# golmschenk/sr-gan

Hardware: AMD Instinct MI355X
Metric: SRGAN train images/sec (G+D step) (higher is better)
Workload: dtype f32; 1 GPU; crowd SRGAN (KnnDenseNetCat D/DNN + DCGenerator) 512x512, batch 16/GPU, dnn_training_step + gan_training_step per step; global_batch=16, image_size=512, schedule=shared-forwards, parallelism=dp1, random_init_weights=True, gradient_penalty=active, launch=eager (Python tape enqueues every kernel), schedule_check=not run: the --full option runs it

## Files before the change

include/srgan_hip.h:

```cpp
#ifndef SRGAN_HIP_H
#define SRGAN_HIP_H

#include <stdint.h>

#ifdef __cplusplus
extern "C" {
#endif

int srgan_version(void);
const char* srgan_build_id(void);
const char* srgan_last_error(void);

#define SRGAN_DTYPE_F32 0x1u
#define SRGAN_DTYPE_BF16 0x2u
#define SRGAN_DTYPE_F16 0x4u
#define SRGAN_FEATURE_FUSED_BNRELU 0x1u
#define SRGAN_FEATURE_SPLITK_WORKSPACE 0x2u
#define SRGAN_FEATURE_LIVE_PROFILE 0x4u
#define SRGAN_FEATURE_BLOCKED16 0x8u
#define SRGAN_FEATURE_BATCHED_SHADOWS 0x10u
#define SRGAN_FEATURE_CROWD_FULL_IMAGE 0x20u
#define SRGAN_FEATURE_IMAGE_BATCHES 0x40u
#define SRGAN_FEATURE_BATCH_NORM_TRAIN 0x80u
#define SRGAN_FEATURE_BLOCKED_BATCH_NORM 0x100u
#define SRGAN_FEATURE_BLOCKED_FROZEN_NORM 0x200u
typedef struct srgan_capabilities_t {
  int32_t abi_version;
  int32_t struct_bytes;
  char arch[16];
  uint32_t dtypes;
  uint32_t features;
  int64_t workspace_bytes;
  int64_t max_tensor_elements;
} srgan_capabilities_t;
int srgan_capabilities(srgan_capabilities_t* out, int32_t out_bytes);
int64_t srgan_workspace_bytes(void);
int srgan_set_workspace(void* workspace, int64_t bytes, void* stream);
int srgan_split_is_ordered(void* stream);

typedef struct srgan_conv_desc {
  int32_t N, C, H, W;
  int32_t K, R, S;
  int32_t stride_h, stride_w, pad_h, pad_w;
  int32_t OH, OW;
  int64_t x_batch_stride, y_batch_stride;
  int32_t compute_dtype;
} srgan_conv_desc;

#define SRGAN_COMPUTE_F32 0
#define SRGAN_COMPUTE_BF16 1
#define SRGAN_COMPUTE_F16 2

int srgan_conv2d_fwd(const srgan_conv_desc* desc, const float* x, const float* w, const float* bias, float* y,
                     int force_kernel, void* stream);

int srgan_conv2d_bwd_data(const srgan_conv_desc* desc, const float* gy, const float* w, const float* bias, float* gx,
                          int accumulate, int force_kernel, void* stream);

// ... 184 lines not shown
int64_t srgan_h_k4s2_weight_slots(int32_t A, int32_t B, int direction, int dtype);
int srgan_h_pack_k4s2_weights(const float* w, void* packed, int32_t A, int32_t B, int direction, int dtype, void* stream);
int32_t srgan_h_pack_job_bytes(void);
int64_t srgan_h_pack_job_conv_weights(void* jobs, int64_t first_block, const float* w, void* packed, int32_t K, int32_t C, int32_t R,
                                      int32_t S, int transposed, int dtype);
int64_t srgan_h_pack_job_k4s2_weights(void* jobs, int64_t first_block, const float* w, void* packed, int32_t A, int32_t B,
                                      int direction, int dtype, int32_t* jobs_written);
int64_t srgan_h_pack_job_matrix(void* jobs, int64_t first_block, const float* src, void* out, int64_t rows, int64_t cols,
                                int64_t rows_real, int64_t cols_real, int64_t row_stride, int64_t col_stride, int32_t row_plane,
                                int32_t col_plane, int dtype);
int64_t srgan_h_pack_job_bias_rows(void* jobs, int64_t first_block, const float* bias, float* rows, int32_t channels, int32_t plane);
int srgan_h_pack_batched(const void* jobs_device, int32_t count, int64_t blocks, void* stream);
int srgan_h_conv4x4s2(const void* x, const void* packed, const float* bias, const void* ref, float slope, int epi, void* out,
                      int32_t N, int32_t C_in, int32_t rows, int32_t H, int32_t W, int dtype, void* stream);
int srgan_h_conv_transpose4x4s2(const void* x, const void* packed, const float* bias, const void* ref, float slope, int epi,
                                void* out, int32_t N, int32_t C_in, int32_t rows, int32_t h, int32_t w, int dtype, void* stream);
int srgan_h_k4s2_wgrad(const void* big, const void* small, float* gw, int32_t N, int32_t C_big, int32_t C_small, int32_t H, int32_t W,
                       int small_is_rows, int dtype, void* stream);

int srgan_h_batch_norm_stats(const void* x, float* mean, float* inv_std, float* running_mean, float* running_var,
                             int64_t* num_batches_tracked, float momentum, float eps, int32_t N, int32_t C, int64_t HW,
                             int32_t dtype, void* stream);
int srgan_h_batch_norm_fwd(const void* x, const float* mean, const float* inv_std, const float* gamma, const float* beta,
                           float slope, void* y, int32_t N, int32_t C, int64_t HW, int32_t dtype, void* stream);
int srgan_h_batch_norm_bwd_reduce(const void* s, const void* x, const float* mean, const float* inv_std, float* sums,
                                  float* g_gamma, float* g_beta, int32_t N, int32_t C, int64_t HW, int32_t dtype, void* stream);
int srgan_h_batch_norm_bwd_apply(const void* s, const void* x, const float* mean, const float* inv_std, const float* gamma,
                                 const float* sums, const void* ref, float slope, void* gx, int32_t N, int32_t C, int64_t HW,
                                 int32_t dtype, void* stream);
int srgan_h_frozen_norm_bwd(const void* s, const void* x, const float* mean, const float* inv_std, const float* gamma,
                            const void* ref, float slope, void* gx, float* g_gamma, float* g_beta, int32_t N, int32_t C, int64_t HW,
                            int32_t dtype, void* stream);

int srgan_profile_begin(void);
int srgan_profile_end(double* kernel_ms, double* flops, double* mfma_flops, int64_t* launches);
int srgan_profile_bytes(double* algorithmic_bytes_total);
int srgan_profile_mixed(double* flops, double* kernel_ms);
int64_t srgan_profile_report(char* buffer, int64_t capacity);

#ifdef __cplusplus
}
#endif
#endif
```

sr-gan_amd/_lib.py:

```python
import ctypes
import os

from ._build import LIBRARY, source_id

c_float_p = ctypes.c_void_p
i32, i64, f32, vp = ctypes.c_int32, ctypes.c_int64, ctypes.c_float, ctypes.c_void_p


class ConvDesc(ctypes.Structure):
    _fields_ = [(name, i32) for name in ('N', 'C', 'H', 'W', 'K', 'R', 'S', 'stride_h', 'stride_w', 'pad_h', 'pad_w',
                                         'OH', 'OW')] + [('x_batch_stride', i64), ('y_batch_stride', i64), ('compute_dtype', i32)]


class BnRelu(ctypes.Structure):
    _fields_ = [(name, vp) for name in ('mean', 'inv_std', 'gamma', 'beta')]


class BnReduceJob(ctypes.Structure):
    _fields_ = [('partial_offset', i64), ('tiles', i32), ('channels', i32), ('inv_std', vp), ('g_gamma', vp), ('g_beta', vp)]


class Capabilities(ctypes.Structure):
    _fields_ = [('abi_version', i32), ('struct_bytes', i32), ('arch', ctypes.c_char * 16), ('dtypes', ctypes.c_uint32),
                ('features', ctypes.c_uint32), ('workspace_bytes', i64), ('max_tensor_elements', i64)]
# ... 84 lines not shown
    'srgan_adam_step': ([vp, vp, vp, vp, i64, f32, f32, f32, f32, f32, i32, vp], ctypes.c_int),
    'srgan_adam_step_counted': ([vp, vp, vp, vp, i64, f32, f32, f32, f32, f32, vp, vp], ctypes.c_int),
    'srgan_pack_bf16': ([vp, vp, i64, vp], ctypes.c_int),
    'srgan_unpack_bf16': ([vp, vp, i64, vp], ctypes.c_int),
    'srgan_h_pack': ([vp, vp, vp, f32, i32, i32, i64, ctypes.c_int, vp], ctypes.c_int),
    'srgan_h_unpack': ([vp, vp, i32, i32, i64, ctypes.c_int, vp], ctypes.c_int),
    'srgan_h_add': ([vp, vp, vp, i64, ctypes.c_int, vp], ctypes.c_int),
    'srgan_h_channel_sums': ([vp, vp, i32, i32, i64, ctypes.c_int, vp], ctypes.c_int),
    'srgan_h_maxpool2': ([vp, vp, vp, i64, i32, i32, ctypes.c_int, ctypes.c_int, vp], ctypes.c_int),
    'srgan_h_maxpool2_bwd': ([vp, vp, vp, i64, i32, i32, ctypes.c_int, f32, ctypes.c_int, vp], ctypes.c_int),
    'srgan_h_conv_weight_slots': ([i32, i32, i32, i32], ctypes.c_int64),
    'srgan_h_pack_conv_weights': ([vp, vp, i32, i32, i32, i32, ctypes.c_int, ctypes.c_int, vp], ctypes.c_int),
    'srgan_h_conv3x3': ([vp, vp, vp, vp, f32, ctypes.c_int, vp, i32, i32, i32, i32, i32, i32, ctypes.c_int, vp], ctypes.c_int),
    'srgan_h_conv3x3_wgrad': ([vp, vp, vp, i32, i32, i32, i32, i32, ctypes.c_int, vp], ctypes.c_int),
    'srgan_h_pack_matrix': ([vp, vp, i64, i64, i64, i64, i64, i64, i32, i32, ctypes.c_int, vp], ctypes.c_int),
    'srgan_h_gemm': ([vp, vp, vp, vp, f32, ctypes.c_int, vp, i32, i32, i32, i32, i32, ctypes.c_int, vp], ctypes.c_int),
    'srgan_h_linear_wgrad': ([vp, vp, vp, i32, i32, i32, i64, i64, i64, i64, i32, i32, ctypes.c_int, vp], ctypes.c_int),
    'srgan_h_k4s2_weight_slots': ([i32, i32, ctypes.c_int, ctypes.c_int], ctypes.c_int64),
    'srgan_h_pack_k4s2_weights': ([vp, vp, i32, i32, ctypes.c_int, ctypes.c_int, vp], ctypes.c_int),
    'srgan_h_pack_job_bytes': ([], ctypes.c_int32),
    'srgan_h_pack_job_conv_weights': ([vp, i64, vp, vp, i32, i32, i32, i32, ctypes.c_int, ctypes.c_int], ctypes.c_int64),
    'srgan_h_pack_job_k4s2_weights': ([vp, i64, vp, vp, i32, i32, ctypes.c_int, ctypes.c_int, vp], ctypes.c_int64),
    'srgan_h_pack_job_matrix': ([vp, i64, vp, vp, i64, i64, i64, i64, i64, i64, i32, i32, ctypes.c_int], ctypes.c_int64),
    'srgan_h_pack_job_bias_rows': ([vp, i64, vp, vp, i32, i32], ctypes.c_int64),
    'srgan_h_pack_batched': ([vp, i32, i64, vp], ctypes.c_int),
    'srgan_h_conv4x4s2': ([vp, vp, vp, vp, f32, ctypes.c_int, vp, i32, i32, i32, i32, i32, ctypes.c_int, vp], ctypes.c_int),
    'srgan_h_conv_transpose4x4s2': ([vp, vp, vp, vp, f32, ctypes.c_int, vp, i32, i32, i32, i32, i32, ctypes.c_int, vp], ctypes.c_int),
    'srgan_h_k4s2_wgrad': ([vp, vp, vp, i32, i32, i32, i32, i32, ctypes.c_int, ctypes.c_int, vp], ctypes.c_int),
    'srgan_h_batch_norm_stats': ([vp, vp, vp, vp, vp, vp, f32, f32, i32, i32, i64, i32, vp], ctypes.c_int),
    'srgan_h_batch_norm_fwd': ([vp, vp, vp, vp, vp, f32, vp, i32, i32, i64, i32, vp], ctypes.c_int),
    'srgan_h_batch_norm_bwd_reduce': ([vp, vp, vp, vp, vp, vp, vp, i32, i32, i64, i32, vp], ctypes.c_int),
    'srgan_h_batch_norm_bwd_apply': ([vp, vp, vp, vp, vp, vp, vp, f32, vp, i32, i32, i64, i32, vp], ctypes.c_int),
    'srgan_h_frozen_norm_bwd': ([vp, vp, vp, vp, vp, vp, f32, vp, vp, vp, i32, i32, i64, i32, vp], ctypes.c_int),
    'srgan_comm_available': ([], ctypes.c_int),
    'srgan_comm_unique_id': ([vp], ctypes.c_int),
    'srgan_comm_init': ([ctypes.POINTER(vp), i32, i32, vp], ctypes.c_int),
    'srgan_comm_world_size': ([vp, ctypes.POINTER(i32)], ctypes.c_int),
    'srgan_comm_destroy': ([vp], ctypes.c_int),
    'srgan_all_reduce_sum': ([vp, vp, vp, i64, i32, vp], ctypes.c_int),
    'srgan_reduce_scatter_sum': ([vp, vp, vp, i64, i32, vp], ctypes.c_int),
    'srgan_all_gather': ([vp, vp, vp, i64, i32, vp], ctypes.c_int),
    'srgan_broadcast': ([vp, vp, i64, i32, i32, vp], ctypes.c_int),
}


EINVAL, EUNSUPPORTED, ERANGE = -1, -2, -3


class HipLibraryError(RuntimeError):

    def __init__(self, message, status=None):
        super().__init__(message)
        self.status = status


_library = None


def library():
    global _library
    if _library is None:
        if not os.path.exists(LIBRARY):
            raise HipLibraryError(f'{LIBRARY} is missing: run `python -c "import __graft_entry__ as g; g.build()"` '
                                  '(there is no CPU fallback)')
        import torch
        lib = ctypes.CDLL(LIBRARY)
# ... 42 lines not shown
```

sr-gan_amd/crowd/models.py:

```python
from collections import OrderedDict

from torch import nn as torch_nn

from .. import functional as F
from .. import nn
from .. import fused
from ..age.models import Generator as _DCGANGenerator, convolution, LEAK
from ..utility import seed_all


FUSED_STEM_POOL = True


class DCGenerator(_DCGANGenerator):

    def __init__(self, z_dim=256, image_size=224, conv_dim=64, batch_norm=None, blocked_batch_norm=False):
        super().__init__(z_dim=z_dim, image_size=image_size, conv_dim=conv_dim, batch_norm=batch_norm,
                         blocked_batch_norm=blocked_batch_norm)


class JointDCDiscriminator(nn.Module):

    def __init__(self, image_size=128, conv_dim=64, number_of_outputs=1):
        seed_all(0)
        super().__init__()
        self.number_of_outputs = number_of_outputs
        self.layer1 = convolution(3, conv_dim, 4, bn=False)
        self.layer2 = convolution(conv_dim, conv_dim * 2, 4)
        self.layer3 = convolution(conv_dim * 2, conv_dim * 4, 4)
        self.layer4 = convolution(conv_dim * 4, conv_dim * 8, 4)
        self.count_layer5 = convolution(conv_dim * 8, self.number_of_outputs, int(image_size / 16), 1, 0, False)
        self.density_layer5 = convolution(conv_dim * 8, int(image_size / 4) ** 2, int(image_size / 16), 1, 0, False)
        self.features = None

    def forward(self, x):
        out = x
        for stage in (self.layer1, self.layer2, self.layer3, self.layer4):
            out = F.leaky_relu(stage(out), LEAK)
        self.features = F.flatten2d(out)
# ... 45 lines not shown
        self.add_module('conv', nn.Conv2d(num_input_features, num_output_features, kernel_size=1, stride=1,
                                          bias=False))
        self.add_module('pool', nn.AvgPool2d(kernel_size=2, stride=2))

    def forward(self, x):
        if fused.POOL_FIRST:
            pooled = None
            if fused.ENABLED and self.pool.kernel_size == 2 and self.pool.stride == 2:
                inv_std, mean = self.norm._inverse_std()
                pooled = F.bn_relu_avg_pool2d(x, mean, inv_std, nn.P(self.norm.weight), nn.P(self.norm.bias))
            if pooled is None:
                pooled = self.pool(self.norm(x, relu=True))
            return self.conv(pooled)
        y = fused.bn_relu_conv(x, self.norm, self.conv) if fused.ENABLED else None
        if y is None:
            y = self.conv(self.norm(x, relu=True))
        return self.pool(y)


class MapModule(nn.Module):

    def __init__(self, in_features, input_size, label_size, count_outputs=1):
        super().__init__()
        kernel_size = label_size // input_size
        self.map_transposed_conv_layer = nn.ConvTranspose2d(in_channels=in_features, out_channels=1,
                                                            kernel_size=kernel_size, stride=kernel_size)
        self.conv1 = nn.Conv2d(in_channels=1, out_channels=8, kernel_size=2, stride=2)
        self.conv2 = nn.Conv2d(in_channels=8, out_channels=16, kernel_size=2, stride=2)
        self.conv3 = nn.Conv2d(in_channels=16, out_channels=32, kernel_size=2, stride=2)
        self.linear1 = nn.Conv2d(in_channels=32, out_channels=20, kernel_size=label_size // (2 ** 3))
        self.count_layer = nn.Conv2d(in_channels=20, out_channels=count_outputs, kernel_size=1)

    def forward(self, x):
        map_ = F.leaky_relu(self.map_transposed_conv_layer(x))
        out = F.leaky_relu(self.conv1(map_))
        out = F.leaky_relu(self.conv2(out))
        out = F.leaky_relu(self.conv3(out))
        out = F.leaky_relu(self.linear1(out))
        return map_, self.count_layer(out), out


class KnnDenseNetCat(nn.Module):

    COUNT_OUTPUTS = 1
    density_is_placeholder = True

    def __init__(self, growth_rate=32, block_config=(6, 12, 48, 32), num_init_features=64, bn_size=4, drop_rate=0,
                 pretrained=False, label_patch_size=224, image_size=None):
        super().__init__()
        image_size = image_size or label_patch_size
        self.label_patch_size = image_size
        self.dense_blocks = nn.ModuleList()
        self.transition_layers = nn.ModuleList()
        self.conv_layer1 = nn.Sequential(OrderedDict([
            ('conv0', nn.Conv2d(3, num_init_features, kernel_size=7, stride=2, padding=3, bias=False)),
            ('norm0', nn.BatchNorm2d(num_init_features)),
            ('relu0', nn.ReLU(inplace=True)),
            ('pool0', nn.MaxPool2d(kernel_size=3, stride=2, padding=1))]))
        num_features = num_init_features
        widths = []
        for i, num_layers in enumerate(block_config):
            block = _DenseBlock(num_layers=num_layers, num_input_features=num_features, bn_size=bn_size,
                                growth_rate=growth_rate, drop_rate=drop_rate)
            self.dense_blocks.add_module('denseblock%d' % (i + 1), block)
            num_features = num_features + num_layers * growth_rate
            if i != len(block_config) - 1:
                self.transition_layers.add_module('transition%d' % (i + 1),
                                                  _Transition(num_features, num_features // 2))
                num_features = num_features // 2
                widths.append(num_features)
        self.norm5 = nn.BatchNorm2d(num_features)
# ... 51 lines not shown

    def _density(self, batch_size, like):
        cache = self._density_cache
        if cache is None or cache.shape[0] != batch_size or cache.data.device != like.data.device:
            cache = F.full((batch_size, self.label_patch_size, self.label_patch_size), 0.0, like)
            self._density_cache = cache
        return cache

    def forward(self, x):
        count, map_, hidden = self._heads(x)
        batch_size = x.shape[0]
        self.features = F.cat_channels([F.view(t, (batch_size, -1, 1, 1)) for t in hidden])
        return self._density(batch_size, x), F.view(count, (batch_size,)), map_

    def _heads(self, x):
        batch_size = x.shape[0]
        stem = self.conv_layer1
        out, first = None, stem.conv0(x)
        if FUSED_STEM_POOL and isinstance(stem.pool0.kernel_size, int):
            inv_std, mean = stem.norm0._inverse_std()
            out = F.bn_relu_max_pool2d(first, mean, inv_std, nn.parameter_var(stem.norm0.weight),
                                       nn.parameter_var(stem.norm0.bias), stem.pool0.kernel_size, stem.pool0.stride,
                                       stem.pool0.padding)
        if out is None:
            out = stem.pool0(stem.norm0(first, relu=True))
        t1_out = self.transition_layers.transition1(self.dense_blocks.denseblock1(out))
        t2_out = self.transition_layers.transition2(self.dense_blocks.denseblock2(t1_out))
        t3_out = self.transition_layers.transition3(self.dense_blocks.denseblock3(t2_out))
        db4_out = self.dense_blocks.denseblock4(t3_out)
        n5_relu_out = self.norm5(db4_out, relu=True)
        final_pool = F.avg_pool2d(n5_relu_out, kernel_size=self.final_pool_size, stride=1)
        final_count_features = F.leaky_relu(self.final_count_feature_layer(final_pool))
        final_count = self.count_layer(final_count_features)
        map1, count1, h1 = self.map_module1(t1_out)
        map2, count2, h2 = self.map_module2(t2_out)
        map3, count3, h3 = self.map_module3(t3_out)
        count = F.add(F.add(F.add(count1, count2), count3), final_count)
        return count, F.cat_channels([map1, map2, map3]), (h1, h2, h3, final_count_features)


class KnnDenseNetCatDggan(KnnDenseNetCat):
    COUNT_OUTPUTS = 2

    def __init__(self, *args, **kwargs):
        super().__init__(*args, **kwargs)
        self.real_label = None

    def forward(self, x):
        outputs, map_, _ = self._heads(x)
        batch_size = x.shape[0]
        self.real_label = F.view(F.slice_channels(outputs, 1, 2), (batch_size,))
        return self._density(batch_size, x), F.view(F.slice_channels(outputs, 0, 1), (batch_size,)), map_
```

sr-gan_amd/csrc/gather_gemm_kernels.hip:

```cpp
#include "common.h"
#include "split_finish.h"
#include "gather_gemm.h"
#include "conv_plan.h"
#include "launchers.h"
#include <stdarg.h>
#include <string.h>
#include <stdlib.h>
#include <atomic>
#include <map>
#include <mutex>
#include <string>
#include <type_traits>
#include <type_traits>
#include <utility>

namespace srgan {

static thread_local char g_error[512] = "";

void set_error(const char* fmt, ...) {
  va_list ap;
  va_start(ap, fmt);
  vsnprintf(g_error, sizeof(g_error), fmt, ap);
  va_end(ap);
// ... 698 lines not shown

int profile_bracket_end(int slot, hipStream_t stream, int64_t M, int64_t N, int64_t K, int kind, int bm, int bn, int split,
                        int akf, int bkf, int64_t b_unique, int precision) {
  if (slot < 0) return SRGAN_OK;
  hipEvent_t stop;
  {
    std::lock_guard<std::mutex> lock(g_profile.mutex);
    if ((size_t)slot >= g_profile.slots) return SRGAN_OK;
    stop = g_profile.events[2 * slot + 1];
    const double f = 2.0 * (double)M * (double)N * (double)K;
    const double bytes = b_unique > 0 ? 4.0 * ((double)M * N + (double)M * K + (double)b_unique)
                                      : algorithmic_bytes((double)M, (double)N, (double)K, kind);
    g_profile.records[slot] = ProfileRecord{(int32_t)M, (int32_t)N, (int32_t)K, kind, bm, bn, split, akf, bkf, bytes, precision};
    g_profile.flops += f;
    if (kind != 0 && kind != 5 && kind != 9 && kind != 12) g_profile.mfma_flops += f;
    g_profile.bytes += bytes;
    g_profile.launches += 1;
  }
  SRGAN_HIP(hipEventRecord(stop, stream));
  return SRGAN_OK;
}

int profile_bracket_end_bytes(int slot, hipStream_t stream, int64_t M, int64_t N, int64_t K, int kind, int bm, int bn, int split,
                              double bytes, int precision) {
  if (slot < 0) return SRGAN_OK;
  hipEvent_t stop;
  {
    std::lock_guard<std::mutex> lock(g_profile.mutex);
    if ((size_t)slot >= g_profile.slots) return SRGAN_OK;
    stop = g_profile.events[2 * slot + 1];
    const double f = 2.0 * (double)M * (double)N * (double)K;
    g_profile.records[slot] = ProfileRecord{(int32_t)M, (int32_t)N, (int32_t)K, kind, bm, bn, split, 0, 0, bytes, precision};
    g_profile.flops += f;
    g_profile.mfma_flops += f;
    g_profile.bytes += bytes;
    g_profile.launches += 1;
  }
  SRGAN_HIP(hipEventRecord(stop, stream));
  return SRGAN_OK;
}

static bool use_pointwise(const ConvGeom& g, int out_channels, int force) {
  const int in_channels = out_channels == g.K ? g.C : g.K;
  const bool plane_ok = g.H * g.W >= 32;
  return force == 0 && pointwise(g) && plane_ok && out_channels >= 8 && in_channels % 2 == 0;
}

static bool use_conv3x3(const ConvGeom& g, int out_channels, int force) {
  return force == 0 && g.R == 3 && g.S == 3 && g.sh == 1 && g.sw == 1 && g.ph == 1 && g.pw == 1 &&
         g.W >= CONV3_MIN_WIDTH && out_channels >= 8;
}

static bool use_conv3x3_mixed(const ConvGeom& g, int out_channels) {
  if (use_conv3x3(g, out_channels, 0)) return true;
  const bool geometry = g.R == 3 && g.S == 3 && g.sh == 1 && g.sw == 1 && g.ph == 1 && g.pw == 1;
  if (!geometry) return false;
  return (g.H == 4 && g.W == 4 && out_channels >= 8) || (g.W >= CONV3_MIN_WIDTH && out_channels >= 1);
}

static bool wgrad3x3_geometry(const ConvGeom& g, int min_width = 7, bool aligned_only = false) {
  const bool aligned = g.W % 4 == 0 && g.x_bs % 4 == 0 && g.y_bs % 4 == 0;
  if (!aligned && aligned_only) return false;
  return g.R == 3 && g.S == 3 && g.sh == 1 && g.sw == 1 && g.ph == 1 && g.pw == 1 && g.W >= min_width && g.C >= 32;
}

static bool use_wgrad3x3(const ConvGeom& g, const float* x, const float* gy, int force) {
  return force == 0 && wgrad3x3_geometry(g);
// ... 447 lines not shown
    const size_t n = out.size() < (size_t)capacity - 1 ? out.size() : (size_t)capacity - 1;
    memcpy(buffer, out.data(), n);
    buffer[n] = 0;
  }
  return (int64_t)out.size() + 1;
}

int64_t srgan_workspace_bytes(void) { return (int64_t)WORKSPACE_BYTES; }

int srgan_set_workspace(void* workspace, int64_t bytes, void* stream) {
  SRGAN_REQUIRE(workspace == nullptr || bytes >= (int64_t)WORKSPACE_BYTES, SRGAN_EINVAL,
                "srgan_set_workspace: at least srgan_workspace_bytes() bytes");
  SRGAN_REQUIRE(((uintptr_t)workspace & 15) == 0, SRGAN_EINVAL, "srgan_set_workspace: 16-byte alignment");
  return workspace_register((float*)workspace, (size_t)(bytes > 0 ? bytes : 0), (hipStream_t)stream);
}

int srgan_split_is_ordered(void* stream) {
  if (split_atomics_forced()) return 0;
  const int set = workspace_index((hipStream_t)stream);
  return set >= 0 && set < SPLIT_TICKET_SETS ? 1 : 0;
}

int srgan_capabilities(srgan_capabilities_t* out, int32_t out_bytes) {
  SRGAN_REQUIRE(out != nullptr && out_bytes >= (int32_t)sizeof(srgan_capabilities_t), SRGAN_EINVAL,
                "srgan_capabilities: output struct");
  memset(out, 0, sizeof(*out));
  out->abi_version = srgan_version();
  out->struct_bytes = (int32_t)sizeof(*out);
  snprintf(out->arch, sizeof(out->arch), "gfx950");
  out->dtypes = SRGAN_DTYPE_F32 | SRGAN_DTYPE_BF16 | SRGAN_DTYPE_F16;
  out->features = SRGAN_FEATURE_FUSED_BNRELU | SRGAN_FEATURE_SPLITK_WORKSPACE | SRGAN_FEATURE_LIVE_PROFILE |
                  SRGAN_FEATURE_BLOCKED16 | SRGAN_FEATURE_BATCHED_SHADOWS | SRGAN_FEATURE_CROWD_FULL_IMAGE |
                  SRGAN_FEATURE_IMAGE_BATCHES | SRGAN_FEATURE_BATCH_NORM_TRAIN | SRGAN_FEATURE_BLOCKED_BATCH_NORM |
                  SRGAN_FEATURE_BLOCKED_FROZEN_NORM;
  out->workspace_bytes = (int64_t)WORKSPACE_BYTES;
  out->max_tensor_elements = ((int64_t)1 << 31) - 1;
  return SRGAN_OK;
}

int srgan_gemm_f32(int32_t M, int32_t N, int32_t K, const float* A, int64_t sai, int64_t sak, const float* B,
                   int64_t sbk, int64_t sbj, float* C, int64_t sci, int64_t scj, const float* bias,
                   int32_t bias_on_columns, int accumulate, int force_kernel, void* stream) {
  return srgan_gemm(M, N, K, A, sai, sak, B, sbk, sbj, C, sci, scj, bias, bias_on_columns, accumulate, force_kernel, 0, stream);
}

int srgan_gemm(int32_t M, int32_t N, int32_t K, const float* A, int64_t sai, int64_t sak, const float* B,
               int64_t sbk, int64_t sbj, float* C, int64_t sci, int64_t scj, const float* bias,
               int32_t bias_on_columns, int accumulate, int force_kernel, int compute_dtype, void* stream) {
  SRGAN_REQUIRE(M > 0 && N > 0 && K >= 0 && A && B && C, SRGAN_EINVAL, "srgan_gemm_f32 arguments");
  SRGAN_REQUIRE(dtype_ok(compute_dtype), SRGAN_EINVAL, "srgan_gemm compute_dtype");
  if (compute_dtype) force_kernel = 2;
  const int64_t lim = (int64_t)1 << 31;
  SRGAN_REQUIRE(M * sai + K * sak < lim && K * sbk + N * sbj < lim && M * sci + N * scj < lim, SRGAN_ERANGE,
                "srgan_gemm_f32 extents");
  SRGAN_REQUIRE((scj == 1 && sci == N) || (sci == 1 && scj == M), SRGAN_EUNSUPPORTED, "srgan_gemm_f32 dense C");
  GatherGemm p = plan_gemm(M, N, K, A, (int32_t)sai, (int32_t)sak, B, (int32_t)sbk, (int32_t)sbj, C, (int32_t)sci,
                           (int32_t)scj, bias, bias_on_columns);
  if (sci == 1 && scj != 1) {
    p = gg_transposed(p);
    choose_staging(p);
  }
  p.precision = compute_dtype;
  std::vector<GatherGemm> plans{p};
  return gg_run_group(plans, C, (int64_t)M * N, accumulate, force_kernel, (hipStream_t)stream);
}

}
// ... 1 lines not shown
```

sr-gan_amd/csrc/launchers.h:

```cpp
#pragma once
#include "common.h"

namespace srgan {

int profile_bracket_begin(hipStream_t stream);
int profile_bracket_end(int slot, hipStream_t stream, int64_t M, int64_t N, int64_t K, int kind, int bm, int bn, int split,
                        int akf = 0, int bkf = 0, int64_t b_unique = 0, int precision = 0);
int profile_bracket_end_bytes(int slot, hipStream_t stream, int64_t M, int64_t N, int64_t K, int kind, int bm, int bn, int split,
                              double bytes, int precision);

struct Conv3Placement { int32_t taps, out_plane, out_sy, out_sx, out_off; };
int conv3x3_splits(int32_t N, int32_t CI, int32_t CO, int32_t H, int32_t W, int precision = 0);
bool conv3x3_epilogue_supported(int32_t N, int32_t CI, int32_t CO, int32_t H, int32_t W);
int64_t conv3x3_epilogue_tiles(int32_t N, int32_t CI, int32_t CO, int32_t H, int32_t W);
int conv3x3_run(const float* in, int64_t in_bs, const float* w, int32_t w_base, int32_t w_so, int32_t w_si, int32_t w_skh,
                int32_t w_skw, const float* bias, float* out, int64_t out_bs, int32_t N, int32_t CI, int32_t CO, int32_t H,
                int32_t W, int accumulate, hipStream_t stream, const float* const* bn = nullptr,
                const BnBackwardEpilogue* epilogue = nullptr, int precision = 0, const Conv3Placement* placement = nullptr);

constexpr int GROUP_OVERSUBSCRIPTION = 4;

int conv3x3_wgrad_run(const float* x, int64_t x_bs, const float* gy, int64_t gy_bs, float* gw, int32_t N, int32_t CI,
                      int32_t CO, int32_t H, int32_t W, int accumulate, hipStream_t stream, const float* const* bn = nullptr,
                      int precision = 0);
// ... 23 lines not shown
                       int tile_pixels, int32_t* rows_done);

bool pointwise_ksplit_wanted(int32_t N, int32_t K, int32_t M, int32_t HW, bool fused_bn);
int pointwise_ksplit_run(const float* in, int64_t in_bs, const float* w, const float* bias, float* out, int64_t out_bs,
                         int32_t N, int32_t K, int32_t M, int32_t HW, int accumulate, hipStream_t stream,
                         const float* const* bn);

bool pointwise_wgrad_enabled();
int pointwise_wgrad_run(const float* x, int64_t x_bs, const float* gy, int64_t gy_bs, float* gw, int32_t N, int32_t CI,
                        int32_t CO, int32_t HW, int accumulate, hipStream_t stream, const float* const* bn = nullptr);
int pointwise_wgrad_group_plan(int64_t x_off, int64_t x_bs, int64_t gy_off, int64_t gy_bs, float* gw, int64_t gw_off, int32_t N, int32_t CI,
                               int32_t CO, int32_t HW, const float* const* bn, int32_t group, int64_t group_weights, int64_t partial_offset,
                               void* job_out, int32_t* grid_x, int32_t* grid_y, int32_t* ragged, int64_t* partial_floats);
int pointwise_wgrad_group_run(const void* jobs, int32_t count, int32_t grid_x, int32_t grid_y, int32_t ragged, int32_t fused_bn,
                              const float* x_base, const float* gy_base, float* gw_base, int64_t flops_mn, int64_t pixels,
                              int64_t elements, int64_t partial_floats, hipStream_t stream);

int bn_train_stats_run(const float* x, float* mean, float* inv_std, float* running_mean, float* running_var,
                       int64_t* num_batches_tracked, float momentum, float eps, int32_t N, int32_t C, int64_t HW,
                       hipStream_t stream);
int bn_train_fwd_run(const float* x, const float* mean, const float* inv_std, const float* gamma, const float* beta, float slope,
                     float* y, int32_t N, int32_t C, int64_t HW, hipStream_t stream);
int bn_train_bwd_reduce_run(const float* g, const float* x, const float* mean, const float* inv_std, const float* gamma,
                            const float* beta, float slope, float* sums, float* g_gamma, float* g_beta, int32_t N, int32_t C,
                            int64_t HW, hipStream_t stream);
int bn_train_bwd_apply_run(const float* g, const float* x, const float* mean, const float* inv_std, const float* gamma,
                           const float* beta, float slope, const float* sums, float* gx, int32_t N, int32_t C, int64_t HW,
                           hipStream_t stream);

int h_frozen_norm_bwd_run(const void* s, const void* x, const float* mean, const float* inv_std, const float* gamma, const void* ref,
                          float slope, void* gx, float* g_gamma, float* g_beta, int32_t N, int32_t C, int64_t HW, int32_t dtype,
                          hipStream_t stream);

bool stem7x7_geometry(int32_t C, int32_t K, int32_t R, int32_t S, int32_t sh, int32_t sw, int32_t ph, int32_t pw);
int stem7x7_fwd_run(const float* x, int64_t x_bs, const float* w, float* y, int64_t y_bs, int32_t N, int32_t H, int32_t W,
                    int32_t K, int32_t OH, int32_t OW, hipStream_t stream);
int stem7x7_wgrad_run(const float* x, int64_t x_bs, const float* gy, int64_t gy_bs, float* gw, int32_t N, int32_t H, int32_t W,
                      int32_t K, int32_t OH, int32_t OW, int accumulate, hipStream_t stream);
int stem7x7_bwd_data_run(const float* gy, int64_t gy_bs, const float* w, float* gx, int64_t gx_bs, int32_t N, int32_t H,
                         int32_t W, int32_t K, int32_t OH, int32_t OW, hipStream_t stream);

}
```

Baseline: 88.07 images/s.

## Fuse the three 2x2-stride map-module conv+leaky chains into one batched kernel

Result: no change. 88.89 images/s (median of 6 runs) (+0.9%).

```diff
diff --git a/include/srgan_hip.h b/include/srgan_hip.h
--- a/include/srgan_hip.h
+++ b/include/srgan_hip.h
@@ -24,6 +24,7 @@
 #define SRGAN_FEATURE_BATCH_NORM_TRAIN 0x80u
 #define SRGAN_FEATURE_BLOCKED_BATCH_NORM 0x100u
 #define SRGAN_FEATURE_BLOCKED_FROZEN_NORM 0x200u
+#define SRGAN_FEATURE_MAP_CHAIN 0x400u
 typedef struct srgan_capabilities_t {
   int32_t abi_version;
   int32_t struct_bytes;
@@ -274,6 +275,11 @@
                             const void* ref, float slope, void* gx, float* g_gamma, float* g_beta, int32_t N, int32_t C, int64_t HW,
                             int32_t dtype, void* stream);
 
+int32_t srgan_map_chain_job_bytes(void);
+int srgan_map_chain_supported(int32_t c0, int32_t c1, int32_t c2, int32_t c3, int32_t S);
+int srgan_map_chain_fwd(const void* jobs, int32_t count, int32_t B, int32_t S, float slope, void* stream);
+int srgan_map_chain_bwd(const void* jobs, int32_t count, int32_t B, int32_t S, float slope, void* stream);
+
 int srgan_profile_begin(void);
 int srgan_profile_end(double* kernel_ms, double* flops, double* mfma_flops, int64_t* launches);
 int srgan_profile_bytes(double* algorithmic_bytes_total);
diff --git a/scratch/kernel_families.py b/scratch/kernel_families.py
--- /dev/null
+++ b/scratch/kernel_families.py
@@ -0,0 +1,38 @@
+import csv
+import re
+import sys
+
+FAMILIES = [('gg_* (contractions)', r'srgan::gg_(?!reduce)'), ('unary_kernel<15>', r'unary_kernel<15>'),
+            ('binary_kernel<6>', r'binary_kernel<6>'), ('chan_reduce_rows_ordered_kernel', r'chan_reduce_rows_ordered_kernel'),
+            ('gg_reduce_partials*', r'gg_reduce_partials'), ('map_chain_fwd_kernel', r'map_chain_fwd'),
+            ('map_chain_bwd_kernel', r'map_chain_bwd')]
+
+
+def read(path):
+    return {row['Name']: (int(row['Calls']), float(row['TotalDurationNs'])) for row in csv.DictReader(open(path))}
+
+
+def per_step(directory, tree):
+    one, three = read(f'{directory}/kernel_stats_1step_{tree}.csv'), read(f'{directory}/kernel_stats_3step_{tree}.csv')
+    rows = {name: [0.0, 0.0] for name, _ in FAMILIES}
+    total = [0.0, 0.0]
+    for kernel, (calls, nanoseconds) in three.items():
+        calls1, nanoseconds1 = one.get(kernel, (0, 0.0))
+        launches, ms = (calls - calls1) / 2, (nanoseconds - nanoseconds1) / 2e6
+        total[0] += launches
+        total[1] += ms
+        for name, pattern in FAMILIES:
+            if re.search(pattern, kernel):
+                rows[name][0] += launches
+                rows[name][1] += ms
+    rows['sum of the families'] = [sum(r[0] for r in rows.values()), sum(r[1] for r in rows.values())]
+    rows['all kernels'] = total
+    return rows
+
+
+directory, trees = sys.argv[1], sys.argv[2:]
+tables = [per_step(directory, tree) for tree in trees]
+print('| family | ' + ' | '.join(f'{tree}: launches / step | {tree}: ms / step' for tree in trees) + ' |')
+print('|---|' + '---|---|' * len(trees))
+for name in tables[0]:
+    print(f'| `{name}` | ' + ' | '.join(f'{table[name][0]:.1f} | {table[name][1]:.3f}' for table in tables) + ' |')
diff --git a/sr-gan_amd/_lib.py b/sr-gan_amd/_lib.py
--- a/sr-gan_amd/_lib.py
+++ b/sr-gan_amd/_lib.py
@@ -140,6 +140,10 @@
     'srgan_h_batch_norm_bwd_reduce': ([vp, vp, vp, vp, vp, vp, vp, i32, i32, i64, i32, vp], ctypes.c_int),
     'srgan_h_batch_norm_bwd_apply': ([vp, vp, vp, vp, vp, vp, vp, f32, vp, i32, i32, i64, i32, vp], ctypes.c_int),
     'srgan_h_frozen_norm_bwd': ([vp, vp, vp, vp, vp, vp, f32, vp, vp, vp, i32, i32, i64, i32, vp], ctypes.c_int),
+    'srgan_map_chain_job_bytes': ([], ctypes.c_int32),
+    'srgan_map_chain_supported': ([i32, i32, i32, i32, i32], ctypes.c_int),
+    'srgan_map_chain_fwd': ([vp, i32, i32, i32, f32, vp], ctypes.c_int),
+    'srgan_map_chain_bwd': ([vp, i32, i32, i32, f32, vp], ctypes.c_int),
     'srgan_comm_available': ([], ctypes.c_int),
     'srgan_comm_unique_id': ([vp], ctypes.c_int),
     'srgan_comm_init': ([ctypes.POINTER(vp), i32, i32, vp], ctypes.c_int),
diff --git a/sr-gan_amd/crowd/map_chain.py b/sr-gan_amd/crowd/map_chain.py
--- /dev/null
+++ b/sr-gan_amd/crowd/map_chain.py
@@ -0,0 +1,148 @@
+import ctypes
+
+from .. import _lib
+from .. import functional as F
+from ..nn import P
+from ..tape import Var, accumulates_into, grad_enabled
+
+ENABLED = True
+
+MAX_JOBS = 4
+SLOT = 16
+STRIDE, PADDING = (2, 2), (0, 0)
+
+
+def composed(map_, module, slope=0.01):
+    out = F.leaky_relu(module.conv1(map_), slope)
+    out = F.leaky_relu(module.conv2(out), slope)
+    return F.leaky_relu(module.conv3(out), slope)
+
+
+def _convs(module):
+    return module.conv1, module.conv2, module.conv3
+
+
+def supported(maps, modules, slope):
+    if not ENABLED or not maps or slope <= 0.0 or F.COMPUTE_DTYPE != 0:
+        return False
+    shape = maps[0].shape
+    if len(shape) != 4 or shape[2] != shape[3]:
+        return False
+    for map_, module in zip(maps, modules):
+        if map_.shape != shape or map_.meta is not None or not map_.data.is_contiguous():
+            return False
+        for conv in _convs(module):
+            if conv.bias is None or tuple(conv.kernel_size) != (2, 2) or tuple(conv.stride) != STRIDE or \
+                    tuple(conv.padding) != PADDING or tuple(conv.dilation) != (1, 1) or conv.groups != 1:
+                return False
+    channels = [modules[0].conv1.in_channels] + [conv.out_channels for conv in _convs(modules[0])]
+    for module in modules:
+        if [module.conv1.in_channels] + [conv.out_channels for conv in _convs(module)] != channels or \
+                [conv.in_channels for conv in _convs(module)] != channels[:3]:
+            return False
+    if shape[1] != channels[0]:
+        return False
+    return bool(_lib.library().srgan_map_chain_supported(*channels, shape[2]))
+
+
+def _launch(name, jobs, batch, side, slope):
+    for first in range(0, len(jobs), MAX_JOBS):
+        group = jobs[first:first + MAX_JOBS]
+        table = (ctypes.c_void_p * (SLOT * len(group)))(*[address for job in group for address in job])
+        F._call(name, table, len(group), batch, side, slope, F._stream())
+
+
+class _Pending:
+
+    def __init__(self, stacked_shape, like):
+        self.grads, self.shape, self.like = {}, stacked_shape, like
+
+    def head_backward(self, index):
+        def backward(g, needs):
+            first = not self.grads
+            self.grads[index] = g
+            return (Var(F._empty(self.shape, self.like)) if first else None,)
+        return backward
+
+    def take(self, heads, head_shape):
+        grads, self.grads = self.grads, {}
+        return [grads[i] if i in grads else F.full(head_shape, 0.0, self.like) for i in range(heads)]
+
+
+def map_chain(maps, modules, slope=0.01):
+    maps, modules = list(maps), list(modules)
+    if not supported(maps, modules, slope):
+        return [composed(map_, module, slope) for map_, module in zip(maps, modules)]
+    heads = len(maps)
+    batch, _, side, _ = maps[0].shape
+    like = maps[0].data
+    widths = [conv.out_channels for conv in _convs(modules[0])]
+    out1 = F._empty((heads, batch, widths[0], side // 2, side // 2), like)
+    out2 = F._empty((heads, batch, widths[1], side // 4, side // 4), like)
+    out3 = F._empty((heads, batch, widths[2], side // 8, side // 8), like)
+    parameters = [[P(tensor) for conv in _convs(module) for tensor in (conv.weight, conv.bias)] for module in modules]
+
+    def job(i, *backward_slots):
+        slots = [maps[i].data.data_ptr()] + [p.data.data_ptr() for p in parameters[i]] + \
+            [out1[i].data_ptr(), out2[i].data_ptr(), out3[i].data_ptr()] + list(backward_slots)
+        return slots + [None] * (SLOT - len(slots))
+    _launch('srgan_map_chain_fwd', [job(i) for i in range(heads)], batch, side, slope)
+
+    inputs = tuple(maps) + tuple(p for head in parameters for p in head)
+    stacked = F._out(out3, inputs, None, 'map_chain')
+    if stacked.node is None:
+        return [Var(out3[i]) for i in range(heads)]
+    pending = _Pending(tuple(out3.shape), like)
+
+    def backward(_, needs):
+        grads = pending.take(heads, tuple(out3.shape[1:]))
+        need_map, need_parameters = needs[:heads], [needs[heads + 6 * i:heads + 6 * i + 6] for i in range(heads)]
+        if grad_enabled():
+            results = [_recorded(i, grads[i], need_map[i], need_parameters[i]) for i in range(heads)]
+            return tuple(r[0] for r in results) + tuple(g for r in results for g in r[1])
+        keep = any(any(row) for row in need_parameters)
+        gmap = F._empty((heads,) + tuple(maps[0].shape), like)
+        kept = [F._empty(t.shape, like) for t in (out1, out2, out3)] if keep else None
+        upstream = [g.data if g.data.is_contiguous() else g.data.contiguous() for g in grads]
+        _launch('srgan_map_chain_bwd',
+                [job(i, upstream[i].data_ptr(), gmap[i].data_ptr(), *([t[i].data_ptr() for t in kept] if keep else []))
+                 for i in range(heads)], batch, side, slope)
+        parameter_grads = []
+        for i in range(heads):
+            layer_inputs = (maps[i].data, out1[i], out2[i])
+            for layer in range(3):
+                weight, bias = parameters[i][2 * layer], parameters[i][2 * layer + 1]
+                need_weight, need_bias = need_parameters[i][2 * layer], need_parameters[i][2 * layer + 1]
+                gw = gb = None
+                if need_weight or need_bias:
+                    x, gy = Var(layer_inputs[layer]), Var(kept[layer][i])
+                if need_weight and accumulates_into(weight):
+                    F._call('srgan_conv2d_bwd_weight', F._conv_desc(x.shape, weight.shape, STRIDE, PADDING, gy.shape), F._ptr(x),
+                            F._ptr(gy), weight.grad_buffer.data_ptr(), 1, F.FORCE_KERNEL, F._stream())
+                elif need_weight:
+                    gw = F.conv2d_backward_weight(x, gy, weight.shape, STRIDE, PADDING)
+                if need_bias and accumulates_into(bias):
+                    F._bias_gradient_into(bias.grad_buffer, gy)
+                elif need_bias:
+                    gb = F.chan_reduce(gy)
+                parameter_grads += [gw, gb]
+        return tuple(Var(gmap[i]) if need_map[i] else None for i in range(heads)) + tuple(parameter_grads)
+
+    def _recorded(i, g, need_map, need_parameters):
+        weights = parameters[i][0::2]
+        if any(need_parameters):
+            from ..tape import backward as sweep
+            wanted = [v for v, need in zip([maps[i]] + parameters[i], [need_map] + list(need_parameters)) if need]
+            found = iter(sweep(composed(maps[i], modules[i], slope), grad=g, inputs=wanted, create_graph=True))
+            values = [next(found) if need else None for need in [need_map] + list(need_parameters)]
+            return values[0], values[1:]
+        if not need_map:
+            return None, [None] * 6
+        saved = (Var(out1[i]), Var(out2[i]), Var(out3[i]))
+        shapes = (maps[i].shape, saved[0].shape, saved[1].shape)
+        for layer in (2, 1, 0):
+            g = F.conv2d_backward_data(F.mask_mul(g, saved[layer], slope), weights[layer], shapes[layer], STRIDE, PADDING)
+        return g, [None] * 6
+
+    stacked.node.backward = backward
+    return [F._out(out3[i], (stacked,), pending.head_backward(i), 'map_chain_head') for i in range(heads)]
diff --git a/sr-gan_amd/crowd/models.py b/sr-gan_amd/crowd/models.py
--- a/sr-gan_amd/crowd/models.py
+++ b/sr-gan_amd/crowd/models.py
@@ -5,6 +5,7 @@
 from .. import functional as F
 from .. import nn
 from .. import fused
+from . import map_chain
 from ..age.models import Generator as _DCGANGenerator, convolution, LEAK
 from ..utility import seed_all
 
@@ -116,11 +117,14 @@
         self.count_layer = nn.Conv2d(in_channels=20, out_channels=count_outputs, kernel_size=1)
 
     def forward(self, x):
-        map_ = F.leaky_relu(self.map_transposed_conv_layer(x))
-        out = F.leaky_relu(self.conv1(map_))
-        out = F.leaky_relu(self.conv2(out))
-        out = F.leaky_relu(self.conv3(out))
-        out = F.leaky_relu(self.linear1(out))
+        map_ = self.map(x)
+        return self.head(map_, map_chain.map_chain([map_], [self])[0])
+
+    def map(self, x):
+        return F.leaky_relu(self.map_transposed_conv_layer(x))
+
+    def head(self, map_, chain_out):
+        out = F.leaky_relu(self.linear1(chain_out))
         return map_, self.count_layer(out), out
 
 
@@ -238,9 +242,11 @@
         final_pool = F.avg_pool2d(n5_relu_out, kernel_size=self.final_pool_size, stride=1)
         final_count_features = F.leaky_relu(self.final_count_feature_layer(final_pool))
         final_count = self.count_layer(final_count_features)
-        map1, count1, h1 = self.map_module1(t1_out)
-        map2, count2, h2 = self.map_module2(t2_out)
-        map3, count3, h3 = self.map_module3(t3_out)
+        modules = (self.map_module1, self.map_module2, self.map_module3)
+        maps = [module.map(t) for module, t in zip(modules, (t1_out, t2_out, t3_out))]
+        chains = map_chain.map_chain(maps, modules)
+        (map1, count1, h1), (map2, count2, h2), (map3, count3, h3) = (
+            module.head(map_, chain) for module, map_, chain in zip(modules, maps, chains))
         count = F.add(F.add(F.add(count1, count2), count3), final_count)
         return count, F.cat_channels([map1, map2, map3]), (h1, h2, h3, final_count_features)
 
diff --git a/sr-gan_amd/csrc/gather_gemm_kernels.hip b/sr-gan_amd/csrc/gather_gemm_kernels.hip
--- a/sr-gan_amd/csrc/gather_gemm_kernels.hip
+++ b/sr-gan_amd/csrc/gather_gemm_kernels.hip
@@ -754,7 +754,7 @@
     const double f = 2.0 * (double)M * (double)N * (double)K;
     g_profile.records[slot] = ProfileRecord{(int32_t)M, (int32_t)N, (int32_t)K, kind, bm, bn, split, 0, 0, bytes, precision};
     g_profile.flops += f;
-    g_profile.mfma_flops += f;
+    if (kind != 25 && kind != 26) g_profile.mfma_flops += f;
     g_profile.bytes += bytes;
     g_profile.launches += 1;
   }
@@ -1268,7 +1268,7 @@
   out->features = SRGAN_FEATURE_FUSED_BNRELU | SRGAN_FEATURE_SPLITK_WORKSPACE | SRGAN_FEATURE_LIVE_PROFILE |
                   SRGAN_FEATURE_BLOCKED16 | SRGAN_FEATURE_BATCHED_SHADOWS | SRGAN_FEATURE_CROWD_FULL_IMAGE |
                   SRGAN_FEATURE_IMAGE_BATCHES | SRGAN_FEATURE_BATCH_NORM_TRAIN | SRGAN_FEATURE_BLOCKED_BATCH_NORM |
-                  SRGAN_FEATURE_BLOCKED_FROZEN_NORM;
+                  SRGAN_FEATURE_BLOCKED_FROZEN_NORM | SRGAN_FEATURE_MAP_CHAIN;
   out->workspace_bytes = (int64_t)WORKSPACE_BYTES;
   out->max_tensor_elements = ((int64_t)1 << 31) - 1;
   return SRGAN_OK;
diff --git a/sr-gan_amd/csrc/launchers.h b/sr-gan_amd/csrc/launchers.h
--- a/sr-gan_amd/csrc/launchers.h
+++ b/sr-gan_amd/csrc/launchers.h
@@ -79,6 +79,9 @@
                           float slope, void* gx, float* g_gamma, float* g_beta, int32_t N, int32_t C, int64_t HW, int32_t dtype,
                           hipStream_t stream);
 
+int map_chain_fwd_run(const void* jobs, int32_t count, int32_t B, int32_t S, float slope, hipStream_t stream);
+int map_chain_bwd_run(const void* jobs, int32_t count, int32_t B, int32_t S, float slope, hipStream_t stream);
+
 bool stem7x7_geometry(int32_t C, int32_t K, int32_t R, int32_t S, int32_t sh, int32_t sw, int32_t ph, int32_t pw);
 int stem7x7_fwd_run(const float* x, int64_t x_bs, const float* w, float* y, int64_t y_bs, int32_t N, int32_t H, int32_t W,
                     int32_t K, int32_t OH, int32_t OW, hipStream_t stream);
diff --git a/sr-gan_amd/csrc/map_chain.hip b/sr-gan_amd/csrc/map_chain.hip
--- /dev/null
+++ b/sr-gan_amd/csrc/map_chain.hip
@@ -0,0 +1,281 @@
+#include "launchers.h"
+
+namespace srgan {
+
+constexpr int MAP_CHAIN_MAX_JOBS = 4;
+constexpr int MAP_CHAIN_THREADS = 256;
+
+struct MapChainJob {
+  const float* map;
+  const float* w1; const float* b1;
+  const float* w2; const float* b2;
+  const float* w3; const float* b3;
+  float* out1; float* out2; float* out3;
+  const float* g3;
+  float* gmap;
+  float* gm1; float* gm2; float* gm3;
+  void* reserved;
+};
+static_assert(sizeof(MapChainJob) == 128, "one job is 16 pointers");
+struct MapChainTable { MapChainJob job[MAP_CHAIN_MAX_JOBS]; };
+
+typedef const float __attribute__((address_space(4)))* uniform_floats;
+__device__ __forceinline__ uniform_floats as_uniform(const float* p) { return (uniform_floats)(uintptr_t)p; }
+
+__device__ __forceinline__ float leaky(float v, float slope) { return v > 0.f ? v : slope * v; }
+__device__ __forceinline__ float masked(float g, float activated, float slope) { return activated > 0.f ? g : slope * g; }
+
+template <int C0, int C1, int C2, int C3>
+__global__ __launch_bounds__(MAP_CHAIN_THREADS) void map_chain_fwd_kernel(const MapChainTable table, int B, int P, float slope) {
+  const MapChainJob& job = table.job[blockIdx.y];
+  const int t = blockIdx.x * MAP_CHAIN_THREADS + threadIdx.x;
+  if (t >= B * P * P) return;
+  const int px = t % P, py = (t / P) % P, b = t / (P * P);
+  const int S = 8 * P, S1 = 4 * P, S2 = 2 * P;
+  const int64_t plane0 = (int64_t)S * S, plane1 = (int64_t)S1 * S1, plane2 = (int64_t)S2 * S2, plane3 = (int64_t)P * P;
+  const float* map = job.map + (int64_t)b * C0 * plane0 + (int64_t)(8 * py) * S + 8 * px;
+  float* out1 = job.out1 + (int64_t)b * C1 * plane1 + (int64_t)(4 * py) * S1 + 4 * px;
+  float* out2 = job.out2 + (int64_t)b * C2 * plane2 + (int64_t)(2 * py) * S2 + 2 * px;
+  float* out3 = job.out3 + (int64_t)b * C3 * plane3 + (int64_t)py * P + px;
+  const uniform_floats w1 = as_uniform(job.w1), b1 = as_uniform(job.b1), w2 = as_uniform(job.w2), b2 = as_uniform(job.b2),
+                       w3 = as_uniform(job.w3), b3 = as_uniform(job.b3);
+
+  float o2[C2][2][2];
+#pragma unroll
+  for (int half = 0; half < 2; ++half) {
+    float m[C0][4][8];
+#pragma unroll
+    for (int c0 = 0; c0 < C0; ++c0)
+#pragma unroll
+      for (int r = 0; r < 4; ++r) {
+        const float* row = map + c0 * plane0 + (int64_t)(4 * half + r) * S;
+        const float4 lo = *reinterpret_cast<const float4*>(row), hi = *reinterpret_cast<const float4*>(row + 4);
+        m[c0][r][0] = lo.x; m[c0][r][1] = lo.y; m[c0][r][2] = lo.z; m[c0][r][3] = lo.w;
+        m[c0][r][4] = hi.x; m[c0][r][5] = hi.y; m[c0][r][6] = hi.z; m[c0][r][7] = hi.w;
+      }
+    float acc2[C2][2];
+#pragma unroll
+    for (int k = 0; k < C2; ++k) acc2[k][0] = acc2[k][1] = b2[k];
+#pragma unroll 1
+    for (int c = 0; c < C1; ++c) {
+      float o1[2][4];
+#pragma unroll
+      for (int r = 0; r < 2; ++r)
+#pragma unroll
+        for (int x = 0; x < 4; ++x) {
+          float v = b1[c];
+#pragma unroll
+          for (int c0 = 0; c0 < C0; ++c0)
+#pragma unroll
+            for (int tap = 0; tap < 4; ++tap)
+              v = fmaf(w1[(c * C0 + c0) * 4 + tap], m[c0][2 * r + (tap >> 1)][2 * x + (tap & 1)], v);
+          o1[r][x] = leaky(v, slope);
+        }
+#pragma unroll
+      for (int r = 0; r < 2; ++r)
+        *reinterpret_cast<float4*>(out1 + c * plane1 + (int64_t)(2 * half + r) * S1) = make_float4(o1[r][0], o1[r][1], o1[r][2], o1[r][3]);
+#pragma unroll
+      for (int k = 0; k < C2; ++k)
+#pragma unroll
+        for (int q = 0; q < 2; ++q)
+#pragma unroll
+          for (int tap = 0; tap < 4; ++tap)
+            acc2[k][q] = fmaf(w2[(k * C1 + c) * 4 + tap], o1[tap >> 1][2 * q + (tap & 1)], acc2[k][q]);
+    }
+#pragma unroll
+    for (int k = 0; k < C2; ++k) {
+      o2[k][half][0] = leaky(acc2[k][0], slope);
+      o2[k][half][1] = leaky(acc2[k][1], slope);
+      *reinterpret_cast<float2*>(out2 + k * plane2 + (int64_t)half * S2) = make_float2(o2[k][half][0], o2[k][half][1]);
+    }
+  }
+#pragma unroll 4
+  for (int k = 0; k < C3; ++k) {
+    float v = b3[k];
+#pragma unroll
+    for (int c = 0; c < C2; ++c)
+#pragma unroll
+      for (int tap = 0; tap < 4; ++tap) v = fmaf(w3[(k * C2 + c) * 4 + tap], o2[c][tap >> 1][tap & 1], v);
+    out3[k * plane3] = leaky(v, slope);
+  }
+}
+
+template <int C0, int C1, int C2, int C3>
+__global__ __launch_bounds__(MAP_CHAIN_THREADS) void map_chain_bwd_kernel(const MapChainTable table, int B, int P, float slope) {
+  const MapChainJob& job = table.job[blockIdx.y];
+  const int t = blockIdx.x * MAP_CHAIN_THREADS + threadIdx.x;
+  if (t >= B * P * P) return;
+  const int px = t % P, py = (t / P) % P, b = t / (P * P);
+  const int S = 8 * P, S1 = 4 * P, S2 = 2 * P;
+  const int64_t plane0 = (int64_t)S * S, plane1 = (int64_t)S1 * S1, plane2 = (int64_t)S2 * S2, plane3 = (int64_t)P * P;
+  const int64_t at0 = (int64_t)b * C0 * plane0 + (int64_t)(8 * py) * S + 8 * px;
+  const int64_t at1 = (int64_t)b * C1 * plane1 + (int64_t)(4 * py) * S1 + 4 * px;
+  const int64_t at2 = (int64_t)b * C2 * plane2 + (int64_t)(2 * py) * S2 + 2 * px;
+  const int64_t at3 = (int64_t)b * C3 * plane3 + (int64_t)py * P + px;
+  const uniform_floats w1 = as_uniform(job.w1), w2 = as_uniform(job.w2), w3 = as_uniform(job.w3);
+  const bool keep = job.gm1 != nullptr;
+
+  float g2[C2][2][2];
+#pragma unroll
+  for (int c = 0; c < C2; ++c) g2[c][0][0] = g2[c][0][1] = g2[c][1][0] = g2[c][1][1] = 0.f;
+  __shared__ float gm3[C3][MAP_CHAIN_THREADS];
+#pragma unroll
+  for (int k = 0; k < C3; ++k) {
+    const float v = masked(job.g3[at3 + k * plane3], job.out3[at3 + k * plane3], slope);
+    gm3[k][threadIdx.x] = v;
+    if (keep) job.gm3[at3 + k * plane3] = v;
+  }
+#pragma unroll 4
+  for (int k = 0; k < C3; ++k) {
+    const float g = gm3[k][threadIdx.x];
+#pragma unroll
+    for (int c = 0; c < C2; ++c)
+#pragma unroll
+      for (int tap = 0; tap < 4; ++tap) g2[c][tap >> 1][tap & 1] = fmaf(w3[(k * C2 + c) * 4 + tap], g, g2[c][tap >> 1][tap & 1]);
+  }
+
+#pragma unroll
+  for (int half = 0; half < 2; ++half) {
+    float gm2[C2][2];
+#pragma unroll
+    for (int k = 0; k < C2; ++k) {
+      const float2 o = *reinterpret_cast<const float2*>(job.out2 + at2 + k * plane2 + (int64_t)half * S2);
+      gm2[k][0] = masked(g2[k][half][0], o.x, slope);
+      gm2[k][1] = masked(g2[k][half][1], o.y, slope);
+    }
+    if (keep) {
+#pragma unroll
+      for (int k = 0; k < C2; ++k)
+        *reinterpret_cast<float2*>(job.gm2 + at2 + k * plane2 + (int64_t)half * S2) = make_float2(gm2[k][0], gm2[k][1]);
+    }
+    float gmap[C0][4][8];
+#pragma unroll
+    for (int c0 = 0; c0 < C0; ++c0)
+#pragma unroll
+      for (int r = 0; r < 4; ++r)
+#pragma unroll
+        for (int x = 0; x < 8; ++x) gmap[c0][r][x] = 0.f;
+#pragma unroll 1
+    for (int c = 0; c < C1; ++c) {
+      float g1[2][4];
+#pragma unroll
+      for (int r = 0; r < 2; ++r)
+#pragma unroll
+        for (int x = 0; x < 4; ++x) g1[r][x] = 0.f;
+#pragma unroll
+      for (int k = 0; k < C2; ++k)
+#pragma unroll
+        for (int q = 0; q < 2; ++q)
+#pragma unroll
+          for (int tap = 0; tap < 4; ++tap)
+            g1[tap >> 1][2 * q + (tap & 1)] = fmaf(w2[(k * C1 + c) * 4 + tap], gm2[k][q], g1[tap >> 1][2 * q + (tap & 1)]);
+#pragma unroll
+      for (int r = 0; r < 2; ++r) {
+        const int64_t row = at1 + c * plane1 + (int64_t)(2 * half + r) * S1;
+        const float4 o = *reinterpret_cast<const float4*>(job.out1 + row);
+        g1[r][0] = masked(g1[r][0], o.x, slope); g1[r][1] = masked(g1[r][1], o.y, slope);
+        g1[r][2] = masked(g1[r][2], o.z, slope); g1[r][3] = masked(g1[r][3], o.w, slope);
+        if (keep) *reinterpret_cast<float4*>(job.gm1 + row) = make_float4(g1[r][0], g1[r][1], g1[r][2], g1[r][3]);
+      }
+#pragma unroll
+      for (int c0 = 0; c0 < C0; ++c0)
+#pragma unroll
+        for (int r = 0; r < 4; ++r)
+#pragma unroll
+          for (int x = 0; x < 8; ++x)
+            gmap[c0][r][x] = fmaf(w1[(c * C0 + c0) * 4 + (r & 1) * 2 + (x & 1)], g1[r >> 1][x >> 1], gmap[c0][r][x]);
+    }
+#pragma unroll
+    for (int c0 = 0; c0 < C0; ++c0)
+#pragma unroll
+      for (int r = 0; r < 4; ++r) {
+        float* row = job.gmap + at0 + c0 * plane0 + (int64_t)(4 * half + r) * S;
+        *reinterpret_cast<float4*>(row) = make_float4(gmap[c0][r][0], gmap[c0][r][1], gmap[c0][r][2], gmap[c0][r][3]);
+        *reinterpret_cast<float4*>(row + 4) = make_float4(gmap[c0][r][4], gmap[c0][r][5], gmap[c0][r][6], gmap[c0][r][7]);
+      }
+  }
+}
+
+static bool aligned16(std::initializer_list<const void*> pointers) {
+  uintptr_t bits = 0;
+  for (const void* p : pointers) {
+    if (!p) return false;
+    bits |= (uintptr_t)p;
+  }
+  return (bits & 15) == 0;
+}
+
+constexpr int C0 = 1, C1 = 8, C2 = 16, C3 = 32;
+constexpr int64_t FMAS_PER_PATCH = 16 * C1 * C0 * 4 + 4 * C2 * C1 * 4 + C3 * C2 * 4;
+constexpr int64_t FLOATS_PER_PATCH = 64 * C0 + 16 * C1 + 4 * C2 + C3;
+
+static int map_chain_arguments(const void* jobs, int32_t count, int32_t B, int32_t S, bool backward, MapChainTable* table) {
+  SRGAN_REQUIRE(jobs && count >= 1 && count <= MAP_CHAIN_MAX_JOBS, SRGAN_EINVAL, "map chain: 1 to 4 jobs per launch");
+  SRGAN_REQUIRE(B > 0 && S > 0 && (S & 7) == 0, SRGAN_EINVAL, "map chain: the map side must be a multiple of 8");
+  SRGAN_REQUIRE((int64_t)B * S * S * 2 * C1 / 8 < ((int64_t)1 << 31), SRGAN_ERANGE, "map chain: tensors are limited to < 2^31 elements");
+  const MapChainJob* source = static_cast<const MapChainJob*>(jobs);
+  for (int i = 0; i < MAP_CHAIN_MAX_JOBS; ++i) {
+    const MapChainJob& job = table->job[i] = source[i < count ? i : 0];
+    if (i >= count) continue;
+    SRGAN_REQUIRE(aligned16({job.map, job.w1, job.b1, job.w2, job.b2, job.w3, job.b3, job.out1, job.out2, job.out3}),
+                  SRGAN_EINVAL, "map chain: every tensor of a job must be given and 16-byte aligned");
+    if (backward) {
+      SRGAN_REQUIRE(aligned16({job.g3, job.gmap}), SRGAN_EINVAL, "map chain backward: g3 and gmap must be given and 16-byte aligned");
+      const bool all = job.gm1 && job.gm2 && job.gm3, none = !job.gm1 && !job.gm2 && !job.gm3;
+      SRGAN_REQUIRE(none || (all && aligned16({job.gm1, job.gm2, job.gm3})), SRGAN_EINVAL,
+                    "map chain backward: the three masked gradients are kept together or not at all, 16-byte aligned");
+    }
+  }
+  return SRGAN_OK;
+}
+
+int map_chain_fwd_run(const void* jobs, int32_t count, int32_t B, int32_t S, float slope, hipStream_t stream) {
+  MapChainTable table;
+  if (const int status = map_chain_arguments(jobs, count, B, S, false, &table)) return status;
+  const int64_t patches = (int64_t)B * (S / 8) * (S / 8);
+  const dim3 grid((unsigned)((patches + MAP_CHAIN_THREADS - 1) / MAP_CHAIN_THREADS), (unsigned)count);
+  const int slot = profile_bracket_begin(stream);
+  hipLaunchKernelGGL((map_chain_fwd_kernel<C0, C1, C2, C3>), grid, dim3(MAP_CHAIN_THREADS), 0, stream, table, B, S / 8, slope);
+  const int status = launch_status();
+  profile_bracket_end_bytes(slot, stream, 1, patches * count, FMAS_PER_PATCH, 25, MAP_CHAIN_THREADS, 1, count,
+                            4.0 * (double)FLOATS_PER_PATCH * (double)(patches * count), 0);
+  return status;
+}
+
+int map_chain_bwd_run(const void* jobs, int32_t count, int32_t B, int32_t S, float slope, hipStream_t stream) {
+  MapChainTable table;
+  if (const int status = map_chain_arguments(jobs, count, B, S, true, &table)) return status;
+  const int64_t patches = (int64_t)B * (S / 8) * (S / 8);
+  const dim3 grid((unsigned)((patches + MAP_CHAIN_THREADS - 1) / MAP_CHAIN_THREADS), (unsigned)count);
+  double floats = 0.0;
+  for (int i = 0; i < count; ++i)
+    floats += (double)(FLOATS_PER_PATCH + C3) + (table.job[i].gm1 ? (double)(16 * C1 + 4 * C2 + C3) : 0.0);
+  const int slot = profile_bracket_begin(stream);
+  hipLaunchKernelGGL((map_chain_bwd_kernel<C0, C1, C2, C3>), grid, dim3(MAP_CHAIN_THREADS), 0, stream, table, B, S / 8, slope);
+  const int status = launch_status();
+  profile_bracket_end_bytes(slot, stream, 1, patches * count, FMAS_PER_PATCH, 26, MAP_CHAIN_THREADS, 1, count,
+                            4.0 * floats * (double)patches, 0);
+  return status;
+}
+
+}
+
+using namespace srgan;
+
+extern "C" {
+
+int32_t srgan_map_chain_job_bytes(void) { return (int32_t)sizeof(MapChainJob); }
+
+int srgan_map_chain_supported(int32_t C0_, int32_t C1_, int32_t C2_, int32_t C3_, int32_t S) {
+  return C0_ == C0 && C1_ == C1 && C2_ == C2 && C3_ == C3 && S > 0 && (S & 7) == 0;
+}
+
+int srgan_map_chain_fwd(const void* jobs, int32_t count, int32_t B, int32_t S, float slope, void* stream) {
+  return map_chain_fwd_run(jobs, count, B, S, slope, (hipStream_t)stream);
+}
+
+int srgan_map_chain_bwd(const void* jobs, int32_t count, int32_t B, int32_t S, float slope, void* stream) {
+  return map_chain_bwd_run(jobs, count, B, S, slope, (hipStream_t)stream);
+}
+
+}
```
